# TAMUCrypto/virgo-plus

Hardware: AMD Instinct MI355X
Metric: prover sec + field-ops/sec, SHA-256 circuit, 1/2/4/8 MI355X (bit-exact) (higher is better)
Workload: dtype u64 (F_p^2, p=2^61-1); 1 GPU; SHA-256 1024-block circuit (SHA256_64.pws x1024, 102347776 gates, 15 layers, 2^23 input wires), GKR sumcheck + Virgo FFT/LDT commit on GPU (BASELINE configs[2]); pass_mode=sync, field_ops_per_proof=8299342697

## Files before the change

virgo-plus_amd/csrc/vp_kernels_pc.h:

```cpp
#pragma once
#include "vp_kernels_round.h"
#include "vp_keccak_asm.h"
#define f_mul f_mul_plain

namespace vp {

__device__ __forceinline__ F root_raw(const F *__restrict__ RT, u32 half_m , u32 e ) { return RT[e & (half_m - 1)]; }
__device__ __forceinline__ F root_fin(const F &r, u32 half_m, u32 e) {
    const bool neg = e >= half_m;
    const u64 nre = r.re ? P61 - r.re : 0, nim = r.im ? P61 - r.im : 0;
    return f_make(neg ? nre : r.re, neg ? nim : r.im);
}
__device__ __forceinline__ F root_pow(const F *__restrict__ RT, u32 half_m, u32 e) { return root_fin(root_raw(RT, half_m, e), half_m, e); }
__device__ __forceinline__ void loads_first() { __builtin_amdgcn_sched_barrier(0); }
__global__ void __launch_bounds__(VP_BLOCK)
k_root_table_step(F *RT, u32 have , F step ) {
    u32 i = blockIdx.x * blockDim.x + threadIdx.x;
    if (i < have) RT[have + i] = f_mul(RT[i], step);
}
__global__ void __launch_bounds__(VP_BLOCK) k_root_compact(const F *__restrict__ RT, u32 stride, u32 n, F *__restrict__ out) {
    const u32 k = blockIdx.x * blockDim.x + threadIdx.x;
    if (k < n) out[k] = RT[(size_t) k * stride];
}

// ... 374 lines not shown
fri_fold_body(const F *__restrict__ in, F *__restrict__ out, u32 Nk, int k, const F *__restrict__ RT, u32 half_m, const F r, F inv2, int lw, u32 rank, u32 live) {
    const size_t t = (size_t) blockIdx.x * blockDim.x + threadIdx.x;
    const u32 No = Nk >> 1;
    if (t >= (size_t) vp_fold_groups(live, VP_FOLD_SPT) * 32 * No) return;
    const u32 al = (u32) (t % No), gb = (u32) (t / No), b = gb & 31, ig = gb >> 5;
    const u32 a = (al << lw) + rank;
    const u32 M = 2 * half_m;
    const u32 e = (u32) ((((unsigned long long) (32 * a + b)) << k) & (M - 1));
    const F inv_mu = root_pow(RT, half_m, e ? M - e : 0);
    F p[VP_FOLD_SPT], q[VP_FOLD_SPT];
#pragma unroll
    for (int j = 0; j < VP_FOLD_SPT; ++j) {
        const size_t sb = (size_t) (ig * VP_FOLD_SPT + j) * 32 + b;
        if (Nk >= 2 && ig * VP_FOLD_SPT + j < live) { p[j] = in[sb * Nk + al]; q[j] = in[sb * Nk + al + No]; }
        else { p[j] = f_zero(); q[j] = f_zero(); }
    }
    loads_first();
    const F c = f_mul(inv2, f_mul(inv_mu, r));
#pragma unroll
    for (int j = 0; j < VP_FOLD_SPT; ++j) {
        const size_t sb = (size_t) (ig * VP_FOLD_SPT + j) * 32 + b;
        if (ig * VP_FOLD_SPT + j < live) out[sb * No + al] = f_add(f_half(f_add(p[j], q[j])), f_mul(c, f_sub(p[j], q[j])));
    }
}
__global__ void __launch_bounds__(VP_BLOCK)
k_fri_fold(const F *__restrict__ in, F *__restrict__ out, u32 Nk, int k, const F *__restrict__ RT, u32 half_m, F r, F inv2, int lw, u32 rank, u32 live) {
    fri_fold_body(in, out, Nk, k, RT, half_m, r, inv2, lw, rank, live);
}
__global__ void __launch_bounds__(VP_BLOCK)
k_fri_fold_p(const F *__restrict__ in, F *__restrict__ out, u32 Nk, int k, const F *__restrict__ RT, u32 half_m, const F *__restrict__ r, F inv2, int lw, u32 rank, u32 live) {
    fri_fold_body(in, out, Nk, k, RT, half_m, *r, inv2, lw, rank, live);
}
#ifndef VP_VO_SPT
#define VP_VO_SPT 4
#endif
__device__ __forceinline__ void
fri_fold0_vo_body(const F *__restrict__ lcw, const F *__restrict__ qcw, const F *__restrict__ hcw, const F *__restrict__ S0, F *__restrict__ out, u32 N,
               const F *__restrict__ RTn , const F *__restrict__ cb , const F r, F half_n ,
               const F *__restrict__ q0, const F *__restrict__ qscal, u32 live ) {
    const size_t t = (size_t) blockIdx.x * blockDim.x + threadIdx.x;
    const u32 No = N >> 1;
    if (t >= (size_t) vp_fold_groups(live, VP_VO_SPT) * 32 * No) return;
    const u32 al = (u32) (t % No), sb = (u32) (t / No), b = sb & 31, ig = sb >> 5;
    const F wa = RTn[(N - al) & (N - 1)];
    F q0a = f_zero(), q0b = f_zero();
    if (q0) { const size_t o = (size_t) b * N + al; q0a = q0[o]; q0b = q0[o + No]; }
    F la[VP_VO_SPT], lb[VP_VO_SPT], ha[VP_VO_SPT], hb[VP_VO_SPT], qa[VP_VO_SPT], qb[VP_VO_SPT];
#pragma unroll
    for (int k = 0; k < VP_VO_SPT; ++k) {
        const size_t p0 = ((size_t) (ig * VP_VO_SPT + k) * 32 + b) * N + al, p1 = p0 + No;
        if (ig * VP_VO_SPT + k < live) {
            la[k] = lcw[p0]; lb[k] = lcw[p1]; ha[k] = hcw[p0]; hb[k] = hcw[p1];
            if (!q0) { qa[k] = qcw[p0]; qb[k] = qcw[p1]; }
        } else la[k] = lb[k] = ha[k] = hb[k] = qa[k] = qb[k] = f_zero();
    }
    loads_first();
    const F inv_x = f_mul(wa, cb[b]);
    const F xn_m1 = cb[32 + b];
    const F xr = f_mul(inv_x, r), hx = f_mul(half_n, inv_x);
#pragma unroll
    for (int k = 0; k < VP_VO_SPT; ++k) {
        const u32 i = ig * VP_VO_SPT + k;
        if (i >= live) continue;
        if (q0) { const F sc = qscal[i]; qa[k] = f_mul(sc, q0a); qb[k] = f_mul(sc, q0b); }
        const F s0 = S0[i];
        const F Ga = f_sub(f_sub(f_mul(la[k], qa[k]), f_mul(xn_m1, ha[k])), s0), Gb = f_sub(f_sub(f_mul(lb[k], qb[k]), f_mul(xn_m1, hb[k])), s0);
        const F D = f_sub(Ga, Gb), S = f_add(Ga, Gb);
        out[((size_t) i * 32 + b) * No + al] = f_mul(hx, f_add(D, f_mul(xr, S)));
    }
}
__global__ void __launch_bounds__(VP_BLOCK)
k_fri_fold0_vo(const F *__restrict__ lcw, const F *__restrict__ qcw, const F *__restrict__ hcw, const F *__restrict__ S0, F *__restrict__ out, u32 N,
               const F *__restrict__ RTn, const F *__restrict__ cb, F r, F half_n, const F *__restrict__ q0, const F *__restrict__ qscal, u32 live) {
    fri_fold0_vo_body(lcw, qcw, hcw, S0, out, N, RTn, cb, r, half_n, q0, qscal, live);
}
__global__ void __launch_bounds__(VP_BLOCK)
k_fri_fold0_vo_p(const F *__restrict__ lcw, const F *__restrict__ qcw, const F *__restrict__ hcw, const F *__restrict__ S0, F *__restrict__ out, u32 N,
                 const F *__restrict__ RTn, const F *__restrict__ cb, const F *__restrict__ r, F half_n, const F *__restrict__ q0, const F *__restrict__ qscal, u32 live) {
    fri_fold0_vo_body(lcw, qcw, hcw, S0, out, N, RTn, cb, *r, half_n, q0, qscal, live);
}
#ifndef VP_VO_GRP
#define VP_VO_GRP 8
#endif
static_assert(64 % (VP_VO_SPT * VP_VO_GRP) == 0, "the 64 slices are dealt to workgroups in groups of VP_VO_SPT * VP_VO_GRP");
template <bool TENSOR, int GRP> __global__ void __launch_bounds__(256)
k_fri_fold0_vo3(const F *__restrict__ lcw, const F *__restrict__ qcw, const F *__restrict__ hcw, const F *__restrict__ S0, F *__restrict__ out1, F *__restrict__ out2,
                F *__restrict__ out3, u32 N, const F *__restrict__ RTn, const F *__restrict__ cb, F r0, F r1, F r2, F half_n, F inv2,
                const F *__restrict__ q0, const F *__restrict__ qscal, u32 live) {
    __shared__ F x1[VP_VO_SPT][2][64], x2[VP_VO_SPT][64];
    const u32 E = N >> 3, No = N >> 1, N2 = N >> 2;
    const u32 lane = threadIdx.x & 63, v = threadIdx.x >> 6;
    const u32 per = E >> 6;
    const u32 al = (blockIdx.x % per) * 64 + lane, sb = blockIdx.x / per, b = sb & 31, ig0 = (sb >> 5) * GRP;
    const u32 a = al + v * E;
    const F inv_x = f_mul(RTn[(N - a) & (N - 1)], cb[b]);
    const F xn_m1 = cb[32 + b];
    const F xr = f_mul(inv_x, r0), hx = f_mul(half_n, inv_x);
    F cA = f_zero(), cB = f_zero(), cC = f_zero(), cE = f_zero(), cK = f_zero();
    if (TENSOR) {
        const size_t o = (size_t) b * N + a;
        const F hxr = f_mul(hx, xr), u = f_add(hx, hxr), w = f_sub(hxr, hx);
        cA = f_mul(u, q0[o]); cB = f_mul(w, q0[o + No]); cC = f_mul(xn_m1, u); cE = f_mul(xn_m1, w); cK = f_add(hxr, hxr);
    }
    const F m1 = f_mul(inv_x, inv_x);
    const F c1 = f_mul(inv2, f_mul(m1, r1));
    const F c2 = f_mul(inv2, f_mul(f_mul(m1, m1), r2));
    const u32 ng = min((u32) GRP, vp_fold_groups(live, VP_VO_SPT) - ig0);
#pragma unroll 1
    for (u32 g = 0; g < ng; ++g) {
        const u32 ig = ig0 + g;
        F la[VP_VO_SPT], lb[VP_VO_SPT], ha[VP_VO_SPT], hb[VP_VO_SPT], qa[VP_VO_SPT], qb[VP_VO_SPT];
#pragma unroll
        for (int k = 0; k < VP_VO_SPT; ++k) {
            const size_t p0 = ((size_t) (ig * VP_VO_SPT + k) * 32 + b) * N + a, p1 = p0 + No;
            if (ig * VP_VO_SPT + k < live) {
                la[k] = lcw[p0]; lb[k] = lcw[p1]; ha[k] = hcw[p0]; hb[k] = hcw[p1];
                if (!TENSOR) { qa[k] = qcw[p0]; qb[k] = qcw[p1]; }
            } else { la[k] = lb[k] = ha[k] = hb[k] = f_zero(); if (!TENSOR) qa[k] = qb[k] = f_zero(); }
        }
        loads_first();
        F f1[VP_VO_SPT];
#pragma unroll
        for (int k = 0; k < VP_VO_SPT; ++k) {
            const u32 i = ig * VP_VO_SPT + k;
            const F s0 = S0[i];
            if (TENSOR) {
                const F X = f_dot2cc(cA, la[k], cB, lb[k]), Y = f_dot2cc(cC, ha[k], cE, hb[k]);
                f1[k] = f_sub(f_dot2cc(qscal[i], X, f_neg(s0), cK), Y);
            } else {
                const F Ga = f_sub(f_sub(f_mul(la[k], qa[k]), f_mul(xn_m1, ha[k])), s0), Gb = f_sub(f_sub(f_mul(lb[k], qb[k]), f_mul(xn_m1, hb[k])), s0);
                const F D = f_sub(Ga, Gb), S = f_add(Ga, Gb);
                f1[k] = f_mul(hx, f_add(D, f_mul(xr, S)));
            }
            if (i < live) out1[((size_t) i * 32 + b) * No + a] = f1[k];
            if (v >= 2) x1[k][v - 2][lane] = f1[k];
        }
        __syncthreads();
        F f2[VP_VO_SPT];
        if (v < 2) {
#pragma unroll
            for (int k = 0; k < VP_VO_SPT; ++k) {
                const u32 i = ig * VP_VO_SPT + k;
                const F gg = x1[k][v][lane];
                f2[k] = f_add(f_half(f_add(f1[k], gg)), f_mul(c1, f_sub(f1[k], gg)));
                if (i < live) out2[((size_t) i * 32 + b) * N2 + a] = f2[k];
                if (v == 1) x2[k][lane] = f2[k];
            }
        }
        __syncthreads();
        if (v == 0) {
#pragma unroll
            for (int k = 0; k < VP_VO_SPT; ++k) {
                const u32 i = ig * VP_VO_SPT + k;
                const F gg = x2[k][lane];
                if (i < live) out3[((size_t) i * 32 + b) * E + al] = f_add(f_half(f_add(f2[k], gg)), f_mul(c2, f_sub(f2[k], gg)));
            }
        }
    }
}
}

namespace vp {

struct SplitArgs {
    const F *in; F *out;
    const F *RT; u32 half_m;
    int ln, l1;
    int inverse;
    u32 in_stride;
    u32 ncoset;
};
template <int L1>
__global__ void __launch_bounds__(VP_BLOCK) k_ntt_split(SplitArgs a) {
    constexpr u32 N1 = 1u << L1;
    const u32 N = 1u << a.ln, N2 = N >> L1, M = 2 * a.half_m;
    const u32 j2 = blockIdx.x * blockDim.x + threadIdx.x, row = blockIdx.y, coset = blockIdx.z;
    if (j2 >= N2) return;
    const u32 wN = M >> a.ln;
    const F *src = a.in + (size_t) row * a.in_stride;
    const bool twist = !a.inverse && coset;
    F x[N1];
#pragma unroll
    for (u32 j1 = 0; j1 < N1; ++j1) {
        F v = src[j1 * N2 + j2];
        if (twist && j1) v = f_mul(v, root_pow(a.RT, a.half_m, (u32) (((unsigned long long) j1 * N2 * coset) & (M - 1))));
        x[j1] = v;
    }
    const bool iota_plus = a.RT[a.half_m >> 1].im == 1;
    const bool ip = a.inverse ? !iota_plus : iota_plus;
#pragma unroll
    for (int s = L1; s >= 1; --s) {
        const u32 half = 1u << (s - 1);
#pragma unroll
        for (u32 idx = 0; idx < N1 / 2; ++idx) {
            const u32 k = idx & (half - 1), i0 = ((idx >> (s - 1)) << s) | k, i1 = i0 + half;
            const u32 e1 = k * (N1 >> s);
            const F u = x[i0], v = x[i1];
            x[i0] = f_add(u, v);
            const F d = f_sub(u, v);
            if (e1 == 0) x[i1] = d;
            else if (4 * e1 == N1) x[i1] = mul_iota(d, ip);
            else {
                u32 e = e1 * (M >> L1);
                if (a.inverse) e = M - e;
                x[i1] = f_mul(d, root_pow(a.RT, a.half_m, e));
            }
        }
    }
    F *dst = a.out + ((size_t) row * a.ncoset + coset) * N;
    const u32 ec = twist ? (u32) (((unsigned long long) j2 * coset) & (M - 1)) : 0u;
    constexpr u32 G = N1 < 4 ? N1 : 4;
#pragma unroll
    for (u32 p0 = 0; p0 < N1; p0 += G) {
        u32 e[G], k1[G]; F w[G];
#pragma unroll
        for (u32 i = 0; i < G; ++i) {
            const u32 p = p0 + i;
            k1[i] = __brev(p) >> (32 - (L1 ? L1 : 1)) >> (L1 ? 0 : 1);
            u32 ee = (u32) (((unsigned long long) j2 * k1[i] * wN) & (M - 1));
            if (a.inverse) ee = ee ? M - ee : 0;
            e[i] = (ee + ec) & (M - 1);
            w[i] = root_raw(a.RT, a.half_m, e[i]);
        }
        loads_first();
#pragma unroll
        for (u32 i = 0; i < G; ++i) {
            const u32 p = p0 + i;
            dst[(size_t) k1[i] * N2 + j2] = (p == 0 && !twist) ? x[p] : f_mul(x[p], root_fin(w[i], a.half_m, e[i]));
        }
    }
}

}

#include "vp_kernels_ntt8.h"
#include "vp_kernels_ntt_long.h"

namespace vp {
#define VP_OPEN_MAX_ORACLES 21
#define VP_OPEN_MAX_PATH 26
struct PcOpenDesc { const F *cw; const F *mask; const Dig *tree; const Dig *top; u32 Nc, n_leaves, n5, lw; };
// ... 186 lines not shown
```

virgo-plus_amd/csrc/vpgpu_fftgkr.inc:

```
namespace {

struct FgkOffsets {
    int lg; u64 r, x, r0, r1, ru_a, rv_a, ru_m, rv_m, dep0, n;
    explicit FgkOffsets(int lg_) : lg(lg_) {
        r = 0; x = lg; r0 = x + 64; r1 = r0 + lg + 10; ru_a = r1 + lg + 10; rv_a = ru_a + lg + 6; ru_m = rv_a + lg + 6; rv_m = ru_m + lg;
        dep0 = rv_m + lg; n = dep0 + (u64) lg * (2 * lg + 2);
    }
    u64 ru_d(int d) const { return dep0 + (u64) d * (2 * lg + 2); }
    u64 rv_d(int d) const { return ru_d(d) + lg; }
    u64 alpha_d(int d) const { return rv_d(d) + lg; }
    u64 beta_d(int d) const { return alpha_d(d) + 1; }
    static u64 n_msgs(int lg) { return 64 + 3ull * (2ull * lg * lg + 2 * lg + 6) + 2 + 2ull * lg; }
};

}

struct FgkState {
    int lg = 0;
    F *B = nullptr, *S = nullptr, *Pm = nullptr, *winv = nullptr, *sq = nullptr, *xsq = nullptr, *g = nullptr, *eu = nullptr, *hi = nullptr, *part = nullptr, *xt = nullptr;
    F *tape = nullptr, *msgs = nullptr;
    Dig *fs_state = nullptr; F *fs_part = nullptr;
    Lane lane;
    std::vector<void *> allocs;
    hipStream_t own_stream = nullptr; hipEvent_t e0 = nullptr, e1 = nullptr, e_dep = nullptr;
// ... 327 lines not shown
    else hipLaunchKernelGGL(k_fg_fs_tail<false>, dim3(1), dim3(VP_BLOCK), lds, st, t);
    prof_end(ctx, st, sl);
    ++ctx->st.launches;
    ctx->st.rounds += rounds;
}

int vp_fft_gkr_fs(vp_ctx *ctx, int lg, const uint8_t state_in[32], vp_F *msgs, uint64_t capacity, uint64_t *n_written, vp_F *tape_out, uint8_t state_out[32]) {
    if (!ctx) return VP_EINVAL;
    VP_ENTER(ctx);
    if (!state_in || !msgs || !tape_out || !state_out) { ctx->err = "vp_fft_gkr_fs: a null argument"; return VP_EINVAL; }
    if (lg < 1 || lg > 19) { ctx->err = "vp_fft_gkr_fs: lg out of range (1..19)"; return VP_ELIMIT; }
    const FgkOffsets o(lg);
    const u64 n_out = FgkOffsets::n_msgs(lg);
    if (capacity < n_out) { ctx->err = "vp_fft_gkr_fs: message buffer size (vp_fft_gkr_sizes)"; return VP_EINVAL; }
    if (ctx->rec) { ctx->err = "vp_fft_gkr_fs: a launch plan is being recorded"; return VP_EINVAL; }
    if (ctx->fgk && ctx->fgk->pending_lg) { ctx->err = "vp_fft_gkr_fs: an asynchronous run is pending (vp_fft_gkr_end / vp_fft_gkr_cancel)"; return VP_EINVAL; }
    VPCHK(fgk_prepare(ctx, lg));
    FgkState &s = *ctx->fgk;
    const hipStream_t st = ctx->stream;
    const u32 N = 1u << lg;
    s.lane.stream = st;
    ctx->st.launches = 0; ctx->st.rounds = 0;
    if (ctx->profiling) ensure_event_pool(ctx);
    ctx->ev_used = 0;
    memcpy(s.h_tape, state_in, 32);
    HIPCHK(hipMemcpyAsync(s.fs_state, s.h_tape, 32, hipMemcpyHostToDevice, st));
    HIPCHK(hipEventRecord(ctx->ev0, st));
    int sl = prof_begin(ctx, st, VP_K_MERKLE, 1, 1, 16ull * (lg + 64), (u64) lg + 64);
    hipLaunchKernelGGL(k_fg_fs_draw, dim3(1), dim3(64), 0, st, s.fs_state, (const F *) nullptr, 0u, s.tape, (u32) o.r, (u32) lg + 64u);
    prof_end(ctx, st, sl);
    VPCHK(fgk_circuit(ctx, s, lg, st));
    sl = prof_begin(ctx, st, VP_K_MERKLE, 1, 1, 16ull * (64 + 2 * (lg + 10)), 64ull + 2 * (lg + 10));
    hipLaunchKernelGGL(k_fg_fs_draw, dim3(1), dim3(64), 0, st, s.fs_state, (const F *) s.msgs, 64u, s.tape, (u32) o.r0, 2u * ((u32) lg + 10u));
    prof_end(ctx, st, sl);
    ctx->st.launches += 2;
    u64 pos = 64;
    hipLaunchKernelGGL(k_fg_gtab, dim3(1), dim3(VP_BLOCK), 0, st, (const F *) (s.tape + o.r0), (const F *) nullptr, 6, (const F *) nullptr, (const F *) nullptr, s.hi);
    hipLaunchKernelGGL(k_fg_add_init, dim3(nblk((u64) 64 * N)), dim3(VP_BLOCK), 0, st, (const F *) s.hi, lg, s.lane.tab[0][1]);
    fgk_fs_sumcheck(ctx, s, st, s.Pm, lg + 6, false, (u32) o.ru_a, s.msgs + pos, (u32) o.rv_a, (u32) lg + 6u);
    pos += 3 * (lg + 6) + 1;
    hipLaunchKernelGGL(k_fg_gtab, dim3(nblk(N)), dim3(VP_BLOCK), 0, st, (const F *) (s.tape + o.ru_a), (const F *) nullptr, lg, (const F *) nullptr, (const F *) nullptr, s.g);
    hipLaunchKernelGGL(k_fg_gtab, dim3(1), dim3(VP_BLOCK), 0, st, (const F *) (s.tape + o.ru_a + lg), (const F *) nullptr, 6, (const F *) nullptr, (const F *) nullptr, s.hi);
    hipLaunchKernelGGL(k_fg_mul_init, dim3(nblk(N)), dim3(VP_BLOCK), 0, st, (const F *) s.g, (const F *) s.hi, (const F *) s.xt, lg, s.lane.tab[0][1]);
    fgk_fs_sumcheck(ctx, s, st, s.S, lg, false, (u32) o.ru_m, s.msgs + pos, (u32) o.rv_m, (u32) lg);
    pos += 3 * lg + 1;
    for (int d = 0; d < lg; ++d) {
        const F *r0 = s.tape + (d ? o.ru_d(d - 1) : o.ru_m), *r1 = s.tape + (d ? o.rv_d(d - 1) : o.rv_m);
        const F *al = d ? s.tape + o.alpha_d(d - 1) : nullptr, *be = d ? s.tape + o.beta_d(d - 1) : nullptr;
        const F *pre = s.B + (size_t) (lg - d - 1) * N;
        hipLaunchKernelGGL(k_fg_gtab, dim3(nblk(N)), dim3(VP_BLOCK), 0, st, r0, r1, lg, al, be, s.g);
        hipLaunchKernelGGL(k_fg_ifft_p1, dim3(nblk(N / 2)), dim3(VP_BLOCK), 0, st, (const F *) s.g, pre, (const F *) s.winv, lg, d, s.lane.tab[0][1], s.lane.tab[0][2]);
        fgk_fs_sumcheck(ctx, s, st, pre, lg, true, (u32) o.ru_d(d), s.msgs + pos, 0u, 0u);
        const F *vu = s.msgs + pos + 3 * lg;
        pos += 3 * lg + 1;
        hipLaunchKernelGGL(k_fg_gtab, dim3(nblk(N)), dim3(VP_BLOCK), 0, st, (const F *) (s.tape + o.ru_d(d)), (const F *) nullptr, lg, (const F *) nullptr, (const F *) nullptr, s.eu);
        hipLaunchKernelGGL(k_fg_ifft_p2, dim3(nblk(N / 2)), dim3(VP_BLOCK), 0, st, (const F *) s.g, (const F *) s.eu, vu, (const F *) s.winv, lg, d, s.lane.tab[0][1], s.lane.tab[0][2]);
        fgk_fs_sumcheck(ctx, s, st, pre, lg, true, (u32) o.rv_d(d), s.msgs + pos, (u32) o.alpha_d(d), 2u);
        pos += 3 * lg + 1;
    }
    if (pos != n_out) { (void) hipStreamSynchronize(st); ctx->err = "internal: fft_gkr message count"; return VP_EINVAL; }
    HIPCHK(hipEventRecord(ctx->ev1, st));
    HIPCHK(hipMemcpyAsync(s.h_msgs, s.msgs, (n_out + o.n + 2) * sizeof(F), hipMemcpyDeviceToHost, st));
    HIPCHK(hipStreamSynchronize(st));
    HIPCHK(hipGetLastError());
    memcpy(msgs, s.h_msgs, n_out * sizeof(F));
    memcpy(tape_out, s.h_msgs + n_out, o.n * sizeof(F));
    memcpy(state_out, s.h_msgs + n_out + o.n, 32);
    float ms = 0;
    hipEventElapsedTime(&ms, ctx->ev0, ctx->ev1);
    ctx->commit_ms = ms;
    if (ctx->profiling) prof_collect(ctx);
    if (n_written) *n_written = n_out;
    return VP_OK;
}

}

static void warm_kernel_functions() {
    static const void *const fns[] = {
        (const void *) k_ntt8_colsx<6>, (const void *) k_ntt8_colsx<7>, (const void *) k_ntt8_colsx<8>, (const void *) k_ntt8_cols<true>, (const void *) k_ntt8_cols<false>,
        (const void *) k_ntt8_rows<true>, (const void *) k_ntt8_rows<false>, (const void *) k_ntt_lds, (const void *) k_leaf_hash<false>, (const void *) k_leaf_hash<true>,
        (const void *) k_leaf_hash_c, (const void *) k_merkle_level, (const void *) k_merkle_top, (const void *) k_pc_products, (const void *) k_pc_quotient, (const void *) k_pc_rank1_check,
        (const void *) k_pc_dot, (const void *) k_pc_sum_parts, (const void *) k_pc_open, (const void *) k_beta_half, (const void *) k_beta_expand, (const void *) k_zero_f,
        (const void *) k_fri_fold, (const void *) k_fri_fold0_vo, (const void *) k_fri_fold0_vo3<true, VP_VO_GRP>, (const void *) k_fri_fold0_vo3<false, VP_VO_GRP>, (const void *) k_fri_fold0_vo3<true, 1>, (const void *) k_fri_fold0_vo3<false, 1>,
        (const void *) k_mask_vo, (const void *) k_fri_fold_one,
        (const void *) k_fg_pows, (const void *) k_fg_expand, (const void *) k_fg_butterfly, (const void *) k_fg_xsq, (const void *) k_fg_xtab, (const void *) k_fg_polyeval,
        (const void *) k_fg_rowsum, (const void *) k_fg_gtab, (const void *) k_fg_add_init, (const void *) k_fg_mul_init, (const void *) k_fg_gtab_multi, (const void *) k_fg_dot_multi,
        (const void *) k_fg_ifft_multi, (const void *) k_fg_ifft_p1, (const void *) k_fg_ifft_p2, (const void *) k_sumfold3b<true>, (const void *) k_sumfold3b<false>,
        (const void *) k_seg<true>, (const void *) k_seg<false>, (const void *) k_emit,
        (const void *) k_fg_fs_draw, (const void *) k_fg_fs_round<true>, (const void *) k_fg_fs_round<false>, (const void *) k_fg_fs_close, (const void *) k_fg_fs_tail<true>, (const void *) k_fg_fs_tail<false>,
        (const void *) k_light_multi, (const void *) k_chunks_multi, (const void *) k_combine_multi, (const void *) k_dot_multi, (const void *) k_dotfin_multi,
        (const void *) k_sumfold3b_multi, (const void *) k_sumfold3b_gen_multi, (const void *) k_seg_multi, (const void *) k_emit_multi, (const void *) k_fixup,
        (const void *) k_beta_half_direct, (const void *) k_beta_half_multi, (const void *) k_vres, (const void *) k_vres2, (const void *) k_tape_in, (const void *) k_ship, (const void *) k_ticket,
        (const void *) k_round_main<0>, (const void *) k_round_main<1>, (const void *) k_round_fused, (const void *) k_round_final, (const void *) k_finalize, (const void *) k_phase,
        (const void *) k_gkr_fs_span, (const void *) k_round_main_fs, (const void *) k_round_fused_fs, (const void *) k_round_final_fs, (const void *) k_gkr_fs_ship,
    };
    for (const void *f : fns) { hipFuncAttributes a; (void) hipFuncGetAttributes(&a, f); }
    (void) hipGetLastError();
}
int vp_warm(vp_ctx *ctx, uint32_t what) {
    if (!ctx || !ctx->evaluated) return VP_EINVAL;
    VP_ENTER(ctx);
    if (what) warm_kernel_functions();
    if (what & VP_WARM_COMMITMENT) VPCHK(pc_warm(ctx));
    if (what & VP_WARM_FFT_GKR) {
        const int lg = ctx->L[0].bl - 6;
        if (lg >= 1 && lg <= 20 && !(ctx->fgk && ctx->fgk->pending_lg) && !ctx->rec) {
            VPCHK(fgk_prepare(ctx, lg));
            if (ctx->opt.fft_gkr_batched) VPCHK(fgk_prepare_batch(ctx, lg));
            FgkState &s = *ctx->fgk;
            if (!s.own_stream) {
                int pr_lo = 0, pr_hi = 0;
                (void) hipDeviceGetStreamPriorityRange(&pr_lo, &pr_hi);
                HIPCHK(hipStreamCreateWithPriority(&s.own_stream, hipStreamNonBlocking, pr_hi));
                HIPCHK(hipEventCreate(&s.e0)); HIPCHK(hipEventCreate(&s.e1));
            }
            if (!s.e_dep) HIPCHK(hipEventCreateWithFlags(&s.e_dep, hipEventDisableTiming));
            {
                const std::vector<vp_F> zero_tape(FgkOffsets(lg).n, vp_F{0, 0});
                VPCHK(fgk_enqueue(ctx, lg, zero_tape.data(), zero_tape.size(), s.own_stream, s.e0, s.e1));
                HIPCHK(hipStreamSynchronize(s.own_stream));
                VPCHK(fgk_enqueue(ctx, lg, zero_tape.data(), zero_tape.size(), ctx->stream, ctx->ev0, ctx->ev1));
                HIPCHK(hipStreamSynchronize(ctx->stream));
                s.lane.stream = ctx->stream;
            }
        }
    }
    return check_stream(ctx);
}
```

virgo-plus_amd/csrc/vpgpu_pc.inc:

```
namespace {

constexpr int PC_MAX_LN = 13;
#ifndef VP_NTT_SPLIT_LOG
#define VP_NTT_SPLIT_LOG 12
#endif
constexpr int PC_SPLIT_LN = VP_NTT_SPLIT_LOG;

#define PC_PROF_IF(on, kind, grid, jobs, bytes, work, ...)                                               \
    do {                                                                                                  \
        const int sl_ = (on) ? prof_begin(ctx, ctx->stream, (kind), (u32) (grid), (u32) (jobs), (u64) (bytes), (u64) (work)) : -1; \
        __VA_ARGS__;                                                                      \
        prof_end(ctx, ctx->stream, sl_);                                                                  \
    } while (0)
#define PC_PROF(kind, grid, jobs, bytes, work, ...) PC_PROF_IF(true, kind, grid, jobs, bytes, work, __VA_ARGS__)

F host_pow(F x, unsigned __int128 e) { F r = f_one(); while (e) { if (e & 1) r = f_mul(r, x); x = f_mul(x, x); e >>= 1; } return r; }
F host_root_of_unity(int log_order) {
    F r = f_make(2147483648ull, 1033321771269002680ull);
    for (int i = 0; i < 62 - log_order; ++i) r = f_mul(r, r);
    return r;
}
F host_inv_real(u64 x) { return host_pow(f_make(x, 0), (unsigned __int128) P61 - 2); }

int pc_root_fill(vp_ctx *ctx, F *rt, int lm) {
// ... 970 lines not shown
    Dig *tree = ctx->pc_fri_tree + fl.tree(k);
    const F *out_m = ctx->pc_mask_ms ? pc_mask_fold(ctx, k, rf, false) : nullptr;
    VPCHK(pc_hash_level(ctx, out, No, out_m, tree));
    HIPCHK(hipEventRecord(ctx->ev1, ctx->stream));
    HIPCHK(hipMemcpyAsync(root, tree + 1, 32, hipMemcpyDeviceToHost, ctx->stream));
    VPCHK(check_stream(ctx));
    ctx->fri_step = k + 1;
    float ms = 0;
    hipEventElapsedTime(&ms, ctx->ev0, ctx->ev1);
    ctx->commit_ms = ms;
    return VP_OK;
}

static int pc_fold0_consts(vp_ctx *ctx, int lm) {
    if (ctx->pc_cbuf_lm == lm) return VP_OK;
    F *cb = nullptr;
    VPCHK(ring_alloc(ctx, 64 * sizeof(F), (void **) &cb));
    const F wM = host_root_of_unity(lm), wMi = host_pow(wM, (unsigned __int128) P61 * P61 - 2), w32 = host_root_of_unity(5);
    F pb = f_one(), pn = f_one();
    for (int b = 0; b < 32; ++b) { cb[b] = pb; cb[32 + b] = f_sub(pn, f_one()); pb = f_mul(pb, wMi); pn = f_mul(pn, w32); }
    HIPCHK(hipMemcpyAsync(ctx->pc_cbuf, cb, 64 * sizeof(F), hipMemcpyHostToDevice, ctx->stream));
    ctx->pc_cbuf_lm = lm;
    return VP_OK;
}

int vp_fri_commit(vp_ctx *ctx, const vp_F *r, int n_steps, uint8_t *roots) {
    if (!ctx || !r || !roots || n_steps < 1) return VP_EINVAL;
    VP_ENTER_Q(ctx);
    if (ctx->pcs) { VPCHK(flush_pending(ctx, (size_t) -1)); return pcs_fri_commit(ctx, r, n_steps, roots); }
    if (!ctx->pc_public_done) return VP_EINVAL;
    const int n = ctx->L[0].bl, ln = n - 6, lm = n - 1;
    const u32 N = 1u << ln, M = 1u << lm;
    if (ctx->fri_step >= 0 && ctx->fri_step != 0) { ctx->err = "vp_fri_commit after vp_fri_step"; return VP_EINVAL; }
    if (n_steps > ln || n_steps > VP_FRI_MAX) { ctx->err = "too many FRI steps"; return VP_EINVAL; }
    const bool masked = ctx->pc_mask_ms != 0;
    if (!ctx->pc_fri_all) {
        VPCHK(dalloc(ctx, &ctx->pc_fri_all, (size_t) 64 * M));
        VPCHK(dalloc(ctx, &ctx->pc_fri_tree, (size_t) M));
    }
    Dig *d_roots = nullptr;
    if (!ctx->pc_fri_roots) VPCHK(dalloc(ctx, &ctx->pc_fri_roots, (size_t) VP_FRI_MAX));
    d_roots = ctx->pc_fri_roots;
    ctx->ev_used = 0;
    hipEvent_t ev_a = nullptr;
    VPCHK(defer_begin(ctx, &ev_a));
    EvGuard ev_guard{ctx, &ev_a};
    ctx->fri_step = 0;
    u32 live = ctx->pc_lv.live;
    VPCHK(pc_live_zero_fri(ctx));
    const FriLayout fl(ln, 0);
    const PcSlices v = pc_slices(ctx, live);
    FriLeafArgs la{}; MerkleArgs ma{};
    if (n_steps + 2 > VP_FRI_MAX) VPCHK(pc_hash_outstanding(ctx, 3u));
    const unsigned merged = ctx->pc_unhashed;
    uint8_t *late_root[2] = {nullptr, nullptr};
    int ne = 0;
    for (int o = 0; o < 2; ++o) {
        if (!(merged >> o & 1)) continue;
        Dig *tree = o ? ctx->pc_tree_h : ctx->pc_tree;
        const u32 n_leaves = M >> 1;
        ma.tree[ne] = tree; ma.count[ne] = n_leaves;
        la.cw[ne] = o ? ctx->pc_hcw : ctx->pc_cw; la.leaves[ne] = tree + n_leaves; la.N[ne] = N;
        if (masked) la.mask[ne] = o ? ctx->pc_hm_cw : ctx->pc_lm_cw;
        late_root[ne] = ctx->late_root[o];
        ++ne;
    }
    const int nt = ne + n_steps;
    const bool fold3 = n_steps >= 3 && ln >= 9;
    for (int k = 0; k < n_steps; ++k) {
        const u32 Nk = N >> k, No = Nk >> 1;
        const F *in = k == 0 ? ctx->pc_qcw : ctx->pc_fri_all + fl.cw(k - 1);
        F *out = ctx->pc_fri_all + fl.cw(k);
        F rf; memcpy(&rf, r + k, sizeof(F));
        if (fold3 && k < 3) {
            if (k == 0) {
                const F *rtn = nullptr;
                VPCHK(pc_circle_roots(ctx, lm, ln, &rtn));
                VPCHK(pc_fold0_consts(ctx, lm));
                F r1, r2; memcpy(&r1, r + 1, sizeof(F)); memcpy(&r2, r + 2, sizeof(F));
                F *o1 = out, *o2 = o1 + (size_t) 64 * 32 * No, *o3 = o2 + (size_t) 64 * 32 * (No >> 1);
                const u32 E = N >> 3;
                const bool grouped = (64 / VP_VO_SPT / VP_VO_GRP) * 32 * (E >> 6) >= 2048;
                const u32 grid3 = vp_fold_groups(live, VP_VO_SPT * (grouped ? VP_VO_GRP : 1)) * 32 * (E >> 6);
                const void *fold3 = v.tensor ? (grouped ? (const void *) k_fri_fold0_vo3<true, VP_VO_GRP> : (const void *) k_fri_fold0_vo3<true, 1>)
                                                     : (grouped ? (const void *) k_fri_fold0_vo3<false, VP_VO_GRP> : (const void *) k_fri_fold0_vo3<false, 1>);
                const F *a_lcw = v.lcw, *a_qcw = v.qcw, *a_hcw = v.hcw, *a_S0 = v.S0(), *a_cb = ctx->pc_cbuf, *a_q0 = v.q0_arg(), *a_qs = v.qs_arg();
                u32 a_N = N;
                F a_half = f_mul(f_make(N, 0), host_inv_real(2)), a_inv2 = host_inv_real(2);
                void *args3[] = {&a_lcw, &a_qcw, &a_hcw, &a_S0, &o1, &o2, &o3, &a_N, &rtn, &a_cb, &rf, &r1, &r2, &a_half, &a_inv2, &a_q0, &a_qs, &live};
                PC_PROF(VP_K_FRI_FOLD, grid3, 1, (v.tensor ? 80ull : 112ull) * live * 32 * No + 16ull * live * 32 * ((No >> 1) + (No >> 2)),
                        (u64) (v.tensor ? 9 : 7) * live * 32 * No + 3ull * live * 32 * ((No >> 1) + (No >> 2)),
                        (void) hipLaunchKernel(fold3, dim3(grid3), dim3(256), args3, 0, ctx->stream));
            }
        }
        else if (k == 0)
        {
            const F *rtn = nullptr;
            VPCHK(pc_circle_roots(ctx, lm, ln, &rtn));
            VPCHK(pc_fold0_consts(ctx, lm));
            PC_PROF(VP_K_FRI_FOLD, nblk((u64) vp_fold_groups(live, VP_VO_SPT) * 32 * No), 1, (v.tensor ? 80ull : 112ull) * live * 32 * No, (u64) (v.tensor ? 9 : 7) * live * 32 * No,
                    hipLaunchKernelGGL(k_fri_fold0_vo, dim3(nblk((u64) vp_fold_groups(live, VP_VO_SPT) * 32 * No)), dim3(VP_BLOCK), 0, ctx->stream, (const F *) v.lcw, (const F *) v.qcw,
                                       (const F *) v.hcw, (const F *) v.S0(), out, N, rtn, (const F *) ctx->pc_cbuf, rf,
                                       f_mul(f_make(N, 0), host_inv_real(2)), v.q0_arg(), v.qs_arg(), live));
        }
        else
        PC_PROF(VP_K_FRI_FOLD, nblk((u64) vp_fold_groups(live, VP_FOLD_SPT) * 32 * No), 1, 48ull * live * 32 * No, (u64) 3 * live * 32 * No,
                hipLaunchKernelGGL(k_fri_fold, dim3(nblk((u64) vp_fold_groups(live, VP_FOLD_SPT) * 32 * No)), dim3(VP_BLOCK), 0, ctx->stream, in, out, Nk, k, ctx->pc_rt, M >> 1, rf,
                                   host_inv_real(2), 0, 0u, live));
        const u32 n_leaves = 16 * No;
        Dig *tree = ctx->pc_fri_tree + fl.tree(k);
        ma.tree[ne + k] = tree; ma.count[ne + k] = n_leaves;
        la.cw[ne + k] = out; la.leaves[ne + k] = tree + n_leaves; la.N[ne + k] = No;
    }
    if (masked) {
        pc_mask_vo(ctx, true);
        for (int k = 0; k < n_steps; ++k) {
            F rf; memcpy(&rf, r + k, sizeof(F));
            la.mask[ne + k] = pc_mask_fold(ctx, k, rf, true);
        }
    }
    la.n = ma.n = nt;
    VPCHK(pc_hash_leaves(ctx, la, true));
    if (merged) { ctx->pc_unhashed = 0; ctx->late_root[0] = ctx->late_root[1] = nullptr; }
    VPCHK(pc_merkle_trees(ctx, ma, d_roots));
    unsigned char *st = nullptr;
    VPCHK(ring_alloc(ctx, (size_t) 32 * nt, (void **) &st));
    HIPCHK(hipMemcpyAsync(st, d_roots, (size_t) 32 * nt, hipMemcpyDeviceToHost, ctx->stream));
    ctx->fri_step = n_steps;
    uint8_t *lr0 = late_root[0], *lr1 = late_root[1];
    return defer_end(ctx, ev_a, VP_PH_FRI, [ctx, st, roots, n_steps, ne, lr0, lr1](float ms) {
        if (ne > 0 && lr0) memcpy(lr0, st, 32);
        if (ne > 1 && lr1) memcpy(lr1, st + 32, 32);
        memcpy(roots, st + 32 * (size_t) ne, (size_t) 32 * n_steps);
        ctx->commit_ms = ms;
        return VP_OK;
    });
}

int vp_fri_commit_fs(vp_ctx *ctx, const uint8_t state_in[32], uint8_t *roots, vp_F *r_out, uint8_t state_out[32]) {
    if (!ctx) return VP_EINVAL;
    VP_ENTER(ctx);
    if (!state_in || !roots || !r_out || !state_out) { ctx->err = "vp_fri_commit_fs: a null argument"; return VP_EINVAL; }
    if (ctx->pcs) { ctx->err = "vp_fri_commit_fs: not built for a sharded commitment (vp_pc_set_shard)"; return VP_EINVAL; }
    if (ctx->L.empty() || !ctx->pc_public_done) { ctx->err = "vp_fri_commit_fs: vp_commit_public first"; return VP_EINVAL; }
    if (ctx->fri_step >= 0) { ctx->err = "vp_fri_commit_fs after vp_fri_step or vp_fri_commit of the same commitment"; return VP_EINVAL; }
    const int n = ctx->L[0].bl, ln = n - 6, lm = n - 1;
    if (ln < 1 || ln > VP_FRI_MAX) { ctx->err = "vp_fri_commit_fs: too many FRI steps"; return VP_ELIMIT; }
    const u32 N = 1u << ln, M = 1u << lm;
    VPCHK(pc_hash_outstanding(ctx, 3u));
    const bool masked = ctx->pc_mask_ms != 0;
    if (!ctx->pc_fri_all) {
        VPCHK(dalloc(ctx, &ctx->pc_fri_all, (size_t) 64 * M));
        VPCHK(dalloc(ctx, &ctx->pc_fri_tree, (size_t) M));
    }
    constexpr size_t FS_DIGS = VP_FRI_MAX + VP_FRI_MAX / 2 + 1;
    if (!ctx->pc_fs) VPCHK(dalloc(ctx, &ctx->pc_fs, FS_DIGS));
    Dig *d_roots = ctx->pc_fs, *d_state = ctx->pc_fs + VP_FRI_MAX + VP_FRI_MAX / 2;
    F *d_r = reinterpret_cast<F *>(ctx->pc_fs + VP_FRI_MAX);
    const F *rtn = nullptr;
    VPCHK(pc_circle_roots(ctx, lm, ln, &rtn));
    VPCHK(pc_fold0_consts(ctx, lm));
    unsigned char *h_in = nullptr, *st = nullptr;
    VPCHK(ring_alloc(ctx, 32, (void **) &h_in));
    VPCHK(ring_alloc(ctx, FS_DIGS * sizeof(Dig), (void **) &st));
    memcpy(h_in, state_in, 32);
    ctx->ev_used = 0;
    hipEvent_t ev_a = nullptr;
    VPCHK(defer_begin(ctx, &ev_a));
// ... 262 lines not shown
```

Measured before the change: 167.4 billion field-ops/s.

## Software-pipeline FRI fold0 vo3 loads with double-buffered slice groups

Restructures the grouped three-level FRI fold kernel so it handles one slice per iteration and prefetches the next group's codeword loads into a second register buffer while the current group computes. Out-of-range slices are clamped instead of branched, and S0/qscal are read through scalar constant-address loads. Launch bounds now request two workgroups per SIMD for the grouped variant. The aim is to hide global-memory latency behind the fold arithmetic and barriers, at the cost of more registers and possible occupancy or spill pressure.

```diff
diff --git a/virgo-plus_amd/csrc/vp_kernels_pc.h b/virgo-plus_amd/csrc/vp_kernels_pc.h
--- a/virgo-plus_amd/csrc/vp_kernels_pc.h
+++ b/virgo-plus_amd/csrc/vp_kernels_pc.h
@@ -480,12 +480,30 @@
 #ifndef VP_VO_GRP
 #define VP_VO_GRP 8
 #endif
+#define VP_VO3_SPT 1
+#define VP_VO3_GRP (VP_VO_SPT * VP_VO_GRP / VP_VO3_SPT)
 static_assert(64 % (VP_VO_SPT * VP_VO_GRP) == 0, "the 64 slices are dealt to workgroups in groups of VP_VO_SPT * VP_VO_GRP");
-template <bool TENSOR, int GRP> __global__ void __launch_bounds__(256)
+static_assert(VP_VO3_SPT * VP_VO3_GRP == VP_VO_SPT * VP_VO_GRP, "the looping form covers the same slices per workgroup");
+__device__ __forceinline__ F f_load_uniform(const F *p) {
+    const __attribute__((address_space(4))) u64 *c = (const __attribute__((address_space(4))) u64 *) p;
+    return f_make(c[0], c[1]);
+}
+template <bool TENSOR, int SPT> __device__ __forceinline__ void
+vo3_request(F (&la)[SPT], F (&lb)[SPT], F (&ha)[SPT], F (&hb)[SPT], F (&qa)[SPT], F (&qb)[SPT] , const F *__restrict__ lcw,
+            const F *__restrict__ qcw, const F *__restrict__ hcw, u32 N, u32 off, u32 ig, u32 live, bool more) {
+    const u32 No = N >> 1, o = more ? off : 0u;
+#pragma unroll
+    for (int k = 0; k < SPT; ++k) {
+        const size_t s = (size_t) (more ? min(ig * SPT + k, live - 1) : 0u) * 32 * N;
+        la[k] = (lcw + s)[o]; lb[k] = (lcw + s)[o + No]; ha[k] = (hcw + s)[o]; hb[k] = (hcw + s)[o + No];
+        if (!TENSOR) { qa[k] = (qcw + s)[o]; qb[k] = (qcw + s)[o + No]; }
+    }
+}
+template <bool TENSOR, int SPT, int GRP> __global__ void __launch_bounds__(256, GRP > 1 ? 2 : 1)
 k_fri_fold0_vo3(const F *__restrict__ lcw, const F *__restrict__ qcw, const F *__restrict__ hcw, const F *__restrict__ S0, F *__restrict__ out1, F *__restrict__ out2,
                 F *__restrict__ out3, u32 N, const F *__restrict__ RTn, const F *__restrict__ cb, F r0, F r1, F r2, F half_n, F inv2,
                 const F *__restrict__ q0, const F *__restrict__ qscal, u32 live) {
-    __shared__ F x1[VP_VO_SPT][2][64], x2[VP_VO_SPT][64];
+    __shared__ F x1[SPT][2][64], x2[SPT][64];
     const u32 E = N >> 3, No = N >> 1, N2 = N >> 2;
     const u32 lane = threadIdx.x & 63, v = threadIdx.x >> 6;
     const u32 per = E >> 6;
@@ -503,58 +521,59 @@
     const F m1 = f_mul(inv_x, inv_x);
     const F c1 = f_mul(inv2, f_mul(m1, r1));
     const F c2 = f_mul(inv2, f_mul(f_mul(m1, m1), r2));
-    const u32 ng = min((u32) GRP, vp_fold_groups(live, VP_VO_SPT) - ig0);
+    const u32 ng = min((u32) GRP, vp_fold_groups(live, SPT) - ig0);
+    const u32 off = b * N + a;
+    F la[2][SPT], lb[2][SPT], ha[2][SPT], hb[2][SPT], qa[2][SPT], qb[2][SPT];
+    auto group = [&](const int h, const u32 ig, const bool ahead, const bool more) __attribute__((always_inline)) {
+            if (ahead) vo3_request<TENSOR, SPT>(la[h ^ 1], lb[h ^ 1], ha[h ^ 1], hb[h ^ 1], qa[h ^ 1], qb[h ^ 1], lcw, qcw, hcw, N, off, ig + 1, live, more);
+            loads_first();
+            F f1[SPT];
+#pragma unroll
+            for (int k = 0; k < SPT; ++k) {
+                const u32 i = ig * SPT + k;
+                const F s0 = f_load_uniform(S0 + i);
+                if (TENSOR) {
+                    const F X = f_dot2cc(cA, la[h][k], cB, lb[h][k]), Y = f_dot2cc(cC, ha[h][k], cE, hb[h][k]);
+                    f1[k] = f_sub(f_dot2cc(f_load_uniform(qscal + i), X, f_neg(s0), cK), Y);
+                } else {
+                    const F Ga = f_sub(f_sub(f_mul(la[h][k], qa[h][k]), f_mul(xn_m1, ha[h][k])), s0), Gb = f_sub(f_sub(f_mul(lb[h][k], qb[h][k]), f_mul(xn_m1, hb[h][k])), s0);
+                    const F D = f_sub(Ga, Gb), S = f_add(Ga, Gb);
+                    f1[k] = f_mul(hx, f_add(D, f_mul(xr, S)));
+                }
+                if (i < live) out1[((size_t) i * 32 + b) * No + a] = f1[k];
+                if (v >= 2) x1[k][v - 2][lane] = f1[k];
+            }
+            __syncthreads();
+            F f2[SPT];
+            if (v < 2) {
+#pragma unroll
+                for (int k = 0; k < SPT; ++k) {
+                    const u32 i = ig * SPT + k;
+                    const F gg = x1[k][v][lane];
+                    f2[k] = f_add(f_half(f_add(f1[k], gg)), f_mul(c1, f_sub(f1[k], gg)));
+                    if (i < live) out2[((size_t) i * 32 + b) * N2 + a] = f2[k];
+                    if (v == 1) x2[k][lane] = f2[k];
+                }
+            }
+            __syncthreads();
+            if (v == 0) {
+#pragma unroll
+                for (int k = 0; k < SPT; ++k) {
+                    const u32 i = ig * SPT + k;
+                    const F gg = x2[k][lane];
+                    if (i < live) out3[((size_t) i * 32 + b) * E + al] = f_add(f_half(f_add(f2[k], gg)), f_mul(c2, f_sub(f2[k], gg)));
+                }
+            }
+    };
+    vo3_request<TENSOR, SPT>(la[0], lb[0], ha[0], hb[0], qa[0], qb[0], lcw, qcw, hcw, N, off, ig0, live, true);
+    if (GRP == 1) { group(0, ig0, false, false); return; }
+    u32 g = 0;
 #pragma unroll 1
-    for (u32 g = 0; g < ng; ++g) {
-        const u32 ig = ig0 + g;
-        F la[VP_VO_SPT], lb[VP_VO_SPT], ha[VP_VO_SPT], hb[VP_VO_SPT], qa[VP_VO_SPT], qb[VP_VO_SPT];
-#pragma unroll
-        for (int k = 0; k < VP_VO_SPT; ++k) {
-            const size_t p0 = ((size_t) (ig * VP_VO_SPT + k) * 32 + b) * N + a, p1 = p0 + No;
-            if (ig * VP_VO_SPT + k < live) {
-                la[k] = lcw[p0]; lb[k] = lcw[p1]; ha[k] = hcw[p0]; hb[k] = hcw[p1];
-                if (!TENSOR) { qa[k] = qcw[p0]; qb[k] = qcw[p1]; }
-            } else { la[k] = lb[k] = ha[k] = hb[k] = f_zero(); if (!TENSOR) qa[k] = qb[k] = f_zero(); }
-        }
-        loads_first();
-        F f1[VP_VO_SPT];
-#pragma unroll
-        for (int k = 0; k < VP_VO_SPT; ++k) {
-            const u32 i = ig * VP_VO_SPT + k;
-            const F s0 = S0[i];
-            if (TENSOR) {
-                const F X = f_dot2cc(cA, la[k], cB, lb[k]), Y = f_dot2cc(cC, ha[k], cE, hb[k]);
-                f1[k] = f_sub(f_dot2cc(qscal[i], X, f_neg(s0), cK), Y);
-            } else {
-                const F Ga = f_sub(f_sub(f_mul(la[k], qa[k]), f_mul(xn_m1, ha[k])), s0), Gb = f_sub(f_sub(f_mul(lb[k], qb[k]), f_mul(xn_m1, hb[k])), s0);
-                const F D = f_sub(Ga, Gb), S = f_add(Ga, Gb);
-                f1[k] = f_mul(hx, f_add(D, f_mul(xr, S)));
-            }
-            if (i < live) out1[((size_t) i * 32 + b) * No + a] = f1[k];
-            if (v >= 2) x1[k][v - 2][lane] = f1[k];
-        }
-        __syncthreads();
-        F f2[VP_VO_SPT];
-        if (v < 2) {
-#pragma unroll
-            for (int k = 0; k < VP_VO_SPT; ++k) {
-                const u32 i = ig * VP_VO_SPT + k;
-                const F gg = x1[k][v][lane];
-                f2[k] = f_add(f_half(f_add(f1[k], gg)), f_mul(c1, f_sub(f1[k], gg)));
-                if (i < live) out2[((size_t) i * 32 + b) * N2 + a] = f2[k];
-                if (v == 1) x2[k][lane] = f2[k];
-            }
-        }
-        __syncthreads();
-        if (v == 0) {
-#pragma unroll
-            for (int k = 0; k < VP_VO_SPT; ++k) {
-                const u32 i = ig * VP_VO_SPT + k;
-                const F gg = x2[k][lane];
-                if (i < live) out3[((size_t) i * 32 + b) * E + al] = f_add(f_half(f_add(f2[k], gg)), f_mul(c2, f_sub(f2[k], gg)));
-            }
-        }
-    }
+    for (; g + 1 < ng; g += 2) {
+        group(0, ig0 + g, true, true);
+        group(1, ig0 + g + 1, true, g + 2 < ng);
+    }
+    if (g < ng) group(0, ig0 + g, false, false);
 }
 }
 
diff --git a/virgo-plus_amd/csrc/vpgpu_fftgkr.inc b/virgo-plus_amd/csrc/vpgpu_fftgkr.inc
--- a/virgo-plus_amd/csrc/vpgpu_fftgkr.inc
+++ b/virgo-plus_amd/csrc/vpgpu_fftgkr.inc
@@ -433,7 +433,7 @@
         (const void *) k_ntt8_rows<true>, (const void *) k_ntt8_rows<false>, (const void *) k_ntt_lds, (const void *) k_leaf_hash<false>, (const void *) k_leaf_hash<true>,
         (const void *) k_leaf_hash_c, (const void *) k_merkle_level, (const void *) k_merkle_top, (const void *) k_pc_products, (const void *) k_pc_quotient, (const void *) k_pc_rank1_check,
         (const void *) k_pc_dot, (const void *) k_pc_sum_parts, (const void *) k_pc_open, (const void *) k_beta_half, (const void *) k_beta_expand, (const void *) k_zero_f,
-        (const void *) k_fri_fold, (const void *) k_fri_fold0_vo, (const void *) k_fri_fold0_vo3<true, VP_VO_GRP>, (const void *) k_fri_fold0_vo3<false, VP_VO_GRP>, (const void *) k_fri_fold0_vo3<true, 1>, (const void *) k_fri_fold0_vo3<false, 1>,
+        (const void *) k_fri_fold, (const void *) k_fri_fold0_vo, (const void *) k_fri_fold0_vo3<true, VP_VO3_SPT, VP_VO3_GRP>, (const void *) k_fri_fold0_vo3<false, VP_VO3_SPT, VP_VO3_GRP>, (const void *) k_fri_fold0_vo3<true, VP_VO_SPT, 1>, (const void *) k_fri_fold0_vo3<false, VP_VO_SPT, 1>,
         (const void *) k_mask_vo, (const void *) k_fri_fold_one,
         (const void *) k_fg_pows, (const void *) k_fg_expand, (const void *) k_fg_butterfly, (const void *) k_fg_xsq, (const void *) k_fg_xtab, (const void *) k_fg_polyeval,
         (const void *) k_fg_rowsum, (const void *) k_fg_gtab, (const void *) k_fg_add_init, (const void *) k_fg_mul_init, (const void *) k_fg_gtab_multi, (const void *) k_fg_dot_multi,
diff --git a/virgo-plus_amd/csrc/vpgpu_pc.inc b/virgo-plus_amd/csrc/vpgpu_pc.inc
--- a/virgo-plus_amd/csrc/vpgpu_pc.inc
+++ b/virgo-plus_amd/csrc/vpgpu_pc.inc
@@ -1076,8 +1076,8 @@
                 const u32 E = N >> 3;
                 const bool grouped = (64 / VP_VO_SPT / VP_VO_GRP) * 32 * (E >> 6) >= 2048;
                 const u32 grid3 = vp_fold_groups(live, VP_VO_SPT * (grouped ? VP_VO_GRP : 1)) * 32 * (E >> 6);
-                const void *fold3 = v.tensor ? (grouped ? (const void *) k_fri_fold0_vo3<true, VP_VO_GRP> : (const void *) k_fri_fold0_vo3<true, 1>)
-                                                     : (grouped ? (const void *) k_fri_fold0_vo3<false, VP_VO_GRP> : (const void *) k_fri_fold0_vo3<false, 1>);
+                const void *fold3 = v.tensor ? (grouped ? (const void *) k_fri_fold0_vo3<true, VP_VO3_SPT, VP_VO3_GRP> : (const void *) k_fri_fold0_vo3<true, VP_VO_SPT, 1>)
+                                                     : (grouped ? (const void *) k_fri_fold0_vo3<false, VP_VO3_SPT, VP_VO3_GRP> : (const void *) k_fri_fold0_vo3<false, VP_VO_SPT, 1>);
                 const F *a_lcw = v.lcw, *a_qcw = v.qcw, *a_hcw = v.hcw, *a_S0 = v.S0(), *a_cb = ctx->pc_cbuf, *a_q0 = v.q0_arg(), *a_qs = v.qs_arg();
                 u32 a_N = N;
                 F a_half = f_mul(f_make(N, 0), host_inv_real(2)), a_inv2 = host_inv_real(2);
```

After: 166.7 billion field-ops/s. Within noise of the previous version (-0.4%).
